# thowell/IterativeLQR.jl

Hardware: AMD Instinct MI355X
Metric: trajectories/sec (whole node), acrobot T=101 batch=1024/GPU (higher is better)
Workload: dtype f64

## Files before the change

iterativelqr.jl_amd/csrc/ilqr_device.hpp:

```cpp
#pragma once

#include <hip/hip_runtime.h>

#include "../../include/ilqr_hip.h"
#include "ilqr_layout.hpp"
#include "ilqr_math.hpp"
#include "ilqr_launch_plan.hpp"
#include "ilqr_ric_schedule.hpp"

namespace ilqr {

struct KArgs {
    double* ws;
    Layout L;
    int B;
    int constrained;
    int stage;
    ilqr_options opt;
    const double* x1;
    const double* u_in;
    double* trace;
    int trace_cap;
    double* qv;
    QLayout QL;
// ... 125 lines not shown
    double *lds;
    double *trace;
    int trace_cap, trace_len;
    double *Q;
    QLayout QL;
    double delta;
    double delta_next;
    int delta_next_ok;
    const double* gzero;
    int T, N, C, lane, wave;
    double objective, max_violation, step_size, gradient_norm;
    int status, iterations, outer_iterations, potrf_info, rollouts, states_eq_nominal;
    int cost_par;
#ifdef ILQR_PROFILE
    double prof[PROF_N];
#endif
};

template <class M> __device__ void gradients_large(Inst<M>& I, bool constrained);
template <class M> __device__ void cost_pass_large(Inst<M>& I, bool at_states, bool upd_J, bool upd_viol, bool constrained, double& J_out, double& viol_out);
template <class M> __device__ void reset_model_objective_large(Inst<M>& I, bool literal);
template <class M, bool STORE_VALUE> __device__ void backward_pass_large(Inst<M>& I);
template <class M> __device__ void rollout_large(Inst<M>& I, double alpha, bool want_delta, double& delta_out);

template <class M, bool STAGE, int NC>
__device__ __forceinline__ double objective_term(double l, const double (&cv)[NC], const double* lam, const double* rho, double* act, bool with_al) {
#pragma clang fp contract(off)
    if (!with_al) return l;
    double dot = 0.0, pen = 0.0;
#pragma unroll
    for (int i = 0; i < NC; ++i) {
        const double lm = lam[i];
        const bool ineq = STAGE ? IneqMask<M>::s(i) : IneqMask<M>::t(i);
        const bool inactive = ineq && cv[i] < 0.0 && lm == 0.0;
        act[i] = inactive ? 0.0 : 1.0;
        dot = __builtin_fma(lm, cv[i], dot);
        const double c2 = cv[i] * cv[i], hr = 0.5 * rho[i];
        if (!inactive) pen = __builtin_fma(hr, c2, pen);
    }
    return (l + dot) + pen;
}
__device__ __forceinline__ void al_multipliers(double rho, double act, double lam, double c, double& ir, double& ct) {
#pragma clang fp contract(off)
    ir = rho * act;
    ct = __builtin_fma(ir, c, lam);
}
struct ObjAcc {
    double a0 = 0.0, a1 = 0.0, a2 = 0.0, a3 = 0.0;
    __device__ __forceinline__ void add(int t, double v) {
        const int q = (t >> 4) & 3;
        a0 += q == 0 ? v : 0.0; a1 += q == 1 ? v : 0.0; a2 += q == 2 ? v : 0.0; a3 += q == 3 ? v : 0.0;
    }
    __device__ __forceinline__ double S() const { return (a0 + a2) + (a1 + a3); }
};

template <class M>
__device__ void cost_pass(Inst<M>& I, const double* X, const double* U, bool upd_J, bool upd_viol,
                          bool constrained, double& J_out, double& viol_out) {
    constexpr int n = M::NX, m = M::NU, ncs = M::NCS, nct = M::NCT;
    ILQR_PROF_BEGIN();
    double Jp = 0.0, vp = 0.0;
    constexpr bool PARK = waves_of<M>::value == 2;
    const int t_first = (PARK && I.wave != 0) ? I.T : I.lane;
    for (int t = t_first; t < I.T; t += 64) {
        double w[cdim<M::NW>::v];
        load_w<M::NW>(I.w, t, w);
        double xt[n];
#pragma unroll
        for (int i = 0; i < n; ++i) xt[i] = X[t * n + i];
        if (t < I.N) {
            double ut[m];
#pragma unroll
            for (int i = 0; i < m; ++i) ut[i] = U[t * m + i];
            double l_ = 0.0;
            if (upd_J) { l_ = M::cost_s(xt, ut, w); ILQR_OPAQUE(l_); }
            if constexpr (ncs == 0) { if (upd_J) Jp += l_; }
            if constexpr (ncs > 0) {
                if (!constrained) { if (upd_J) Jp += l_; }
                if (constrained) {
                    double cv[ncs];
                    M::con_s(xt, ut, w, cv);
                    const int off = t * ncs;
                    if (upd_J) { double v_ = objective_term<M, true, ncs>(l_, cv, I.lam + off, I.rho + off, I.act + off, true); ILQR_OPAQUE(v_); Jp += v_; }
                    if (upd_viol) {
#pragma unroll
                        for (int i = 0; i < ncs; ++i) {
                            I.c[off + i] = cv[i];
                            const bool ineq = IneqMask<M>::s(i);
                            vp = nanmax(vp, ineq ? nanmax(0.0, cv[i]) : fabs(cv[i]));
                        }
                    }
                }
            }
        } else {
            double l_ = 0.0;
            if (upd_J) { l_ = M::cost_t(xt, w); ILQR_OPAQUE(l_); }
            if constexpr (nct == 0) { if (upd_J) Jp += l_; }
            if constexpr (nct > 0) {
                if (!constrained) { if (upd_J) Jp += l_; }
                if (constrained) {
                    double cv[nct];
                    M::con_t(xt, w, cv);
                    const int off = I.N * ncs;
                    if (upd_J) { double v_ = objective_term<M, false, nct>(l_, cv, I.lam + off, I.rho + off, I.act + off, true); ILQR_OPAQUE(v_); Jp += v_; }
                    if (upd_viol) {
#pragma unroll
                        for (int i = 0; i < nct; ++i) {
                            I.c[off + i] = cv[i];
                            const bool ineq = IneqMask<M>::t(i);
                            vp = nanmax(vp, ineq ? nanmax(0.0, cv[i]) : fabs(cv[i]));
                        }
                    }
                }
            }
        }
    }
    if constexpr (PARK) {
        double* hand = I.zs + 8 + 2 * I.cost_par;
        I.cost_par ^= 1;
        if (I.wave == 0) {
            J_out = wave_sum(Jp);
            viol_out = wave_max(vp);
            if (I.lane == 0) { hand[0] = J_out; hand[1] = viol_out; }
        }
        __syncthreads();
        if (I.wave != 0) { J_out = hand[0]; viol_out = hand[1]; }
    } else {
        J_out = wave_sum(Jp);
        viol_out = wave_max(vp);
        __syncthreads();
    }
#ifndef ILQR_PROFILE_BAR
    ILQR_PROF_END(I, PROF_COST);
#endif
}

template <class M>
__device__ void cost_bang(Inst<M>& I, bool mode_current, bool constrained) {
    const bool one_pass = mode_current || I.states_eq_nominal || !constrained;
    const int npass = one_pass ? 1 : 2;
    for (int pass = 0; pass < npass; ++pass) {
        const bool at_states = mode_current || pass == 1;
        const bool upd_J = pass == 0;
        const bool upd_viol = one_pass || pass == 1;
        double J, v;
        if constexpr (is_large<M>::value) cost_pass_large<M>(I, at_states, upd_J, upd_viol, constrained, J, v);
        else cost_pass<M>(I, at_states ? I.x : I.xb, at_states ? I.u : I.ub, upd_J, upd_viol, constrained, J, v);
        if (upd_J) I.objective = J;
        if (upd_viol && constrained) I.max_violation = v;
    }
}

template <class M>
__device__ void gradients_small(Inst<M>& I, bool constrained) {
    constexpr int n = M::NX, m = M::NU, ncs = M::NCS, nct = M::NCT, W = waves_of<M>::value;
    ILQR_PROF_BEGIN();
    for (int t = I.lane + 64 * I.wave; t < I.T; t += 64 * W) {
        double w[cdim<M::NW>::v];
        load_w<M::NW>(I.w, t, w);
        double xt[n];
#pragma unroll
        for (int i = 0; i < n; ++i) xt[i] = I.xb[t * n + i];
        if (t < I.N) {
            double ut[m];
#pragma unroll
            for (int i = 0; i < m; ++i) ut[i] = I.ub[t * m + i];
            {
                double fx[n * n], fu[n * m];
                M::dyn_jac(xt, ut, w, fx, fu);
#pragma unroll
                for (int i = 0; i < n * n; ++i) I.fx[t * n * n + i] = fx[i];
#pragma unroll
                for (int i = 0; i < n * m; ++i) I.fu[t * n * m + i] = fu[i];
            }
            double gx[n], gu[m];
            M::cost_s_grad(xt, ut, w, gx, gu);
            if constexpr (ncs == 0) {
                M::cost_s_hess_acc(xt, ut, w, I.gxx + t * n * n, I.guu + t * m * m, I.gux + t * m * n);
#pragma unroll
                for (int i = 0; i < n; ++i) I.gx[t * n + i] = gx[i];
#pragma unroll
                for (int i = 0; i < m; ++i) I.gu[t * m + i] = gu[i];
                continue;
            }
            M::cost_s_hess_acc(xt, ut, w, I.gxx + t * n * n, I.guu + t * m * m, I.gux + t * m * n);
            if constexpr (ncs > 0) {
                if (constrained) {
                    double ct[ncs], ir[ncs];
                    const int off = t * ncs;
#pragma unroll
                    for (int i = 0; i < ncs; ++i) al_multipliers(I.rho[off + i], I.act[off + i], I.lam[off + i], I.c[off + i], ir[i], ct[i]);
                    M::al_s(xt, ut, w, ct, ir, gx, gu, I.gxx + t * n * n, I.guu + t * m * m, I.gux + t * m * n);
                }
            }
#pragma unroll
            for (int i = 0; i < n; ++i) I.gx[t * n + i] = gx[i];
#pragma unroll
            for (int i = 0; i < m; ++i) I.gu[t * m + i] = gu[i];
        } else {
            double gx[n];
            M::cost_t_grad(xt, w, gx);
            M::cost_t_hess_acc(xt, w, I.gxx + t * n * n);
            if constexpr (nct > 0) {
                if (constrained) {
                    double ct[nct], ir[nct];
                    const int off = I.N * ncs;
#pragma unroll
                    for (int i = 0; i < nct; ++i) al_multipliers(I.rho[off + i], I.act[off + i], I.lam[off + i], I.c[off + i], ir[i], ct[i]);
                    M::al_t(xt, w, ct, ir, gx, I.gxx + t * n * n);
                }
            }
#pragma unroll
            for (int i = 0; i < n; ++i) I.gx[t * n + i] = gx[i];
        }
    }
    __syncthreads();
    ILQR_PROF_END(I, PROF_GRAD);
}

template <int m>
__device__ __forceinline__ int potrf_U(double (&A)[m * m], double (&R)[m]) {
    int info = 0;
#pragma unroll
    for (int j = 0; j < m; ++j) {
        double ajj = A[j * m + j];
#pragma unroll
        for (int l = 0; l < j; ++l) ajj -= A[j * m + l] * A[j * m + l];
        const bool ok = (info == 0) && (ajj > 0.0);
        const bool fail_now = (info == 0) && !(ajj > 0.0);
        info = fail_now ? j + 1 : info;
        double dq, rq;
        sqrt_rsqrt_fast(ok ? ajj : 1.0, dq, rq);
        const double dbad = fail_now ? ajj : A[j * m + j];
        const double d = ok ? dq : dbad;
        A[j * m + j] = d;
        double r = rq;
        if (__builtin_expect(!ok, 0)) r = 1.0 / dbad;
        R[j] = r;
#pragma unroll
        for (int c = j + 1; c < m; ++c) {
            double v = A[c * m + j];
#pragma unroll
            for (int l = 0; l < j; ++l) v -= A[j * m + l] * A[c * m + l];
            A[c * m + j] = ok ? v * r : A[c * m + j];
        }
    }
    return info;
}
template <int m>
__device__ __forceinline__ int potrf_U(double (&A)[m * m]) {
    double R[m];
    return potrf_U<m>(A, R);
}
template <int m>
__device__ __forceinline__ bool potrf_U_nofail(double (&A)[m * m], double (&R)[m]) {
    bool bad = false;
#pragma unroll
    for (int j = 0; j < m; ++j) {
        double ajj = A[j * m + j];
#pragma unroll
        for (int l = 0; l < j; ++l) ajj -= A[j * m + l] * A[j * m + l];
        bad |= !(ajj > 0.0);
        double dq, rq;
        sqrt_rsqrt_fast(ajj, dq, rq);
        A[j * m + j] = dq;
        R[j] = rq;
#pragma unroll
        for (int c = j + 1; c < m; ++c) {
            double v = A[c * m + j];
#pragma unroll
            for (int l = 0; l < j; ++l) v -= A[j * m + l] * A[c * m + l];
            A[c * m + j] = v * rq;
        }
    }
    return bad;
}
template <int m, int nrhs>
__device__ __forceinline__ void potrs_U_rdiag(const double (&U)[m * m], const double (&R)[m], double (&B)[m * nrhs]) {
#pragma unroll
    for (int c = 0; c < nrhs; ++c) {
#pragma unroll
        for (int i = 0; i < m; ++i) {
            double v = B[c * m + i];
#pragma unroll
            for (int l = 0; l < i; ++l) v -= U[i * m + l] * B[c * m + l];
            B[c * m + i] = v * R[i];
        }
#pragma unroll
        for (int i = m - 1; i >= 0; --i) {
            double v = B[c * m + i];
#pragma unroll
            for (int l = i + 1; l < m; ++l) v -= U[l * m + i] * B[c * m + l];
            B[c * m + i] = v * R[i];
        }
    }
}
template <int m, int nrhs>
__device__ __forceinline__ void potrs_U(const double (&U)[m * m], double (&B)[m * nrhs]) {
#pragma unroll
    for (int c = 0; c < nrhs; ++c) {
#pragma unroll
        for (int i = 0; i < m; ++i) {
            double v = B[c * m + i];
#pragma unroll
            for (int l = 0; l < i; ++l) v -= U[i * m + l] * B[c * m + l];
            B[c * m + i] = v / U[i * m + i];
        }
#pragma unroll
        for (int i = m - 1; i >= 0; --i) {
            double v = B[c * m + i];
#pragma unroll
            for (int l = i + 1; l < m; ++l) v -= U[l * m + i] * B[c * m + l];
            B[c * m + i] = v / U[i * m + i];
        }
    }
}

__device__ __forceinline__ double lane_bcast(double v, int src_lane) {
    int lo = __double2loint(v), hi = __double2hiint(v);
    lo = __builtin_amdgcn_readlane(lo, src_lane);
    hi = __builtin_amdgcn_readlane(hi, src_lane);
    return __hiloint2double(hi, lo);
}
__device__ __forceinline__ double row_from_next_quad(double v) {
    int lo = __double2loint(v), hi = __double2hiint(v), olo, ohi;
    asm volatile("s_nop 7\n\ts_nop 7\n\tv_mov_b32_dpp %0, %2 row_shl:4 row_mask:0xf bank_mask:0xf bound_ctrl:1\n\t"
                 "v_mov_b32_dpp %1, %3 row_shl:4 row_mask:0xf bank_mask:0xf bound_ctrl:1\n\ts_nop 1"
// ... 570 lines not shown
        }
        return __builtin_amdgcn_ballot_w64(!(qmin > 0.0) || P != P) != 0;
    } else {
        unsigned agx = vr ? lds(I.gx + tl * n + r) : zero;             const unsigned dgx = vr ? 32u * n : 0u;
        unsigned agu = lds(I.gu + tl);
        unsigned aK = vr ? lds(I.K + tl * n + r) : zero;
        unsigned arq = vr ? lds(I.ring + M1_RQ + r) : zero;            const unsigned dq = vr ? 32u * n : 0u;
        unsigned asa = lds(I.ring + M1_RS);
        unsigned ak = lds(I.k + tl);
        asm volatile("" : "+v"(agu), "+v"(asa), "+v"(ak));
        unsigned oLu = goff(I.gbase + I.hLu + tl);
        unsigned oLx = vr ? goff(I.gbase + I.hLx + tl * n + r) : goff(I.gzero + 2 + GZERO_REGION);   const unsigned dLx = vr ? 32u * n : 0u;
        auto GS = [&](unsigned o, int off, double v) { *(double*)(const_cast<char*>(gb) + (size_t)o + (ptrdiff_t)(8 * off)) = v; };
        double p = vr ? I.gx[N * n + r] : 0.0;
        if (STORE_VALUE && b0 && vr && c == 0) I.p[N * n + r] = p;
        double gmax = 0.0, nu = 0.0, dacc = 0.0;
        unsigned long long nanmask = 0;
        auto fetch = [&](Opnd& o, int i) {
            o.fx = LD(afx, i * n * n); o.fu = LD(afu, i * n);
            o.c0 = LD(agx, i * n); o.c1 = LD(agu, i);
        };
        auto step = [&](const Opnd& o, int i) {
            ILQR_ISA_MARK("riccati_step", ROLE);
            const double Qx = mfma444(o.fx, p, o.c0);
            const double Qu = mfma444(o.fu, p, o.c1);
            const double sa = LD(asa, i * n);
            const double Kc = LD(aK, i * n), Quxc = LD(arq, i * n), uxtc = LD(arq, M1_RU - M1_RQ + i * n);
            const double k = (Qu * sa) * -1.0;
            const double pn = fma(uxtc, k, fma(Quxc, k, fma(Kc, Qu, Qx)));
            const double Lx = Qx - pn;
            asm("v_max_f64 %0, %1, |%2|" : "=v"(gmax) : "v"(gmax), "v"(Lx));
            asm("v_max_f64 %0, %1, |%2| ; %3" : "=v"(gmax) : "v"(gmax), "v"(Qu), "v"(Lx));
            nanmask |= __builtin_amdgcn_ballot_w64(__builtin_isunordered(Lx, Qu));
            ST(ak, i, k); GS(oLu, i, Qu); GS(oLx, i * n, Lx);
            const double wv = mfma444(o.fu, nu, Qu);
            dacc = fma(wv, k, dacc);
            const double nun = mfma444(o.fx, nu, Lx);
            nu = fma(Kc, wv, nun);
            if constexpr (STORE_VALUE) {
                if (b0 && c == 0) {
                    if (vr) I.p[t * n + r] = pn;
                    if (I.Q != nullptr) {
                        if (vr) I.Q[I.QL.Qx + t * n + r] = Qx;
                        if (r == 0) I.Q[I.QL.Qu + t] = Qu;
                    }
                }
            }
            p = pn;
            --t;
        };
        if (t0 & 1) fetch(A, t0 & 3); else fetch(B, t0 & 3);
        for (int e = t0 & 3;; e = 3) {
            ILQR_BAR_BEGIN();
            __syncthreads();
            ILQR_BAR_END(I, PROF_COST);
            switch (e) {
                case 3: fetch(B, 2); step(A, 3); [[fallthrough]];
                case 2: fetch(A, 1); step(B, 2); [[fallthrough]];
                case 1: fetch(B, 0); step(A, 1); [[fallthrough]];
                default:
                    afx -= dfx; afu -= dfu; agx -= dgx; agu -= 32u;
                    fetch(A, 3); step(B, 0);
            }
            aK -= dq; ak -= 32u; oLu -= 32u; oLx -= dLx;
            arq += par ? (0u - dq) : dq;
            asa += par ? (unsigned)(-32 * n) : 32u * n;
            par ^= 1;
            asm volatile("" : "+v"(afx), "+v"(afu), "+v"(agx), "+v"(agu), "+v"(aK), "+v"(ak), "+v"(arq), "+v"(asa));
            if (t < 0) break;
        }
        I.gradient_norm = wave_max(nanmask != 0 ? __builtin_nan("") : gmax);
        I.delta_next = lane_bcast(dacc, 0);
#ifdef ILQR_PROFILE_BAR
        if (lane == 0) I.zs[7] += I.prof[PROF_COST];
        I.prof[PROF_COST] = 0.0;
#endif
        return false;
    }
}

template <class M, bool STORE_VALUE>
__device__ __forceinline__ void backward_pass(Inst<M>& I) {
    ILQR_PROF_BEGIN();
    if constexpr (is_large<M>::value) backward_pass_large<M, STORE_VALUE>(I);
    else {
        if constexpr (waves_of<M>::value == 1) {
            backward_pass_mfma<M, STORE_VALUE, 0>(I);
            __syncthreads();
        } else {
            bool literal = true;
            if constexpr (M::NU == 1) {
                if (I.wave == 0) {
                    const bool bad = backward_pass_m1<M, STORE_VALUE, 1>(I);
                    if (I.lane == 0) { I.zs[6] = bad ? 1.0 : 0.0; I.zs[3] = (double)I.potrf_info; }
                } else {
                    backward_pass_m1<M, STORE_VALUE, 2>(I);
                    if (I.lane == 0) { I.zs[2] = I.gradient_norm; I.zs[5] = I.delta_next; }
                }
                __syncthreads();
                literal = I.zs[6] != 0.0;
#ifdef ILQR_PROFILE
                if (literal) I.prof[PROF_DELTA] += 1.0;
#endif
                if (literal) {
                    if (I.wave == 0 && I.lane == 0) I.scal[S_LITERAL_PASSES] += 1.0;
                    __syncthreads();
                }
            }
            if (literal) {
                if (I.wave == 0) {
                    backward_pass_split<M, STORE_VALUE, 1>(I);
                    if (I.lane == 0) I.zs[3] = (double)I.potrf_info;
                } else {
                    backward_pass_split<M, STORE_VALUE, 2>(I);
                    if (I.lane == 0) { I.zs[2] = I.gradient_norm; I.zs[5] = I.delta_next; }
                }
                __syncthreads();
                if constexpr (lagrangian_home_is_hbm<M>::value) {
                    for (int i = threadIdx.x; i < I.N * M::NX; i += 128) I.gbase[I.hLx + i] = I.Lx[i];
                    for (int i = threadIdx.x; i < I.N * M::NU; i += 128) I.gbase[I.hLu + i] = I.Lu[i];
                }
            }
            I.gradient_norm = I.zs[2]; I.potrf_info = (int)I.zs[3];
            I.delta_next = I.zs[5]; I.delta_next_ok = 1;
        }
    }
    ILQR_PROF_END(I, PROF_BACKWARD);
}

template <class M, bool MULTI = false>
__device__ void rollout_small(Inst<M>& I, double alpha, bool with_delta, double& delta_out, int nt = 1, double* buf1 = nullptr,
                              int xs = 0, int bsz = 0) {
    constexpr int n = M::NX, m = M::NU;
    constexpr bool MF = (n <= 4 && m <= 4) && waves_of<M>::value == 1;
    constexpr bool PRE = (m <= n);
    typedef __attribute__((address_space(3))) double ldsd;
    const int lane = I.lane;
    double* xr = I.x; double* ur = I.u;
    const double alpha0 = alpha;
    (void)alpha0;
    if constexpr (MULTI) {
        const int jr = (lane >> 4) < nt - 1 ? (lane >> 4) : nt - 1;
        if (jr > 0) { xr = buf1 + (jr - 1) * bsz; ur = xr + xs; }
        for (int j = 0; j < jr; ++j) alpha *= 0.5;
    }
    if constexpr (PRE) {
        for (int t = lane; t < I.N; t += 64) {
#pragma unroll
            for (int i = 0; i < m; ++i) {
                double b = 0.0;
#pragma unroll
                for (int j = 0; j < n; ++j) b = fma(I.K[t * m * n + j * m + i], I.xb[t * n + j], b);
                if constexpr (MULTI) {
                    double al = alpha0;
                    for (int j = 0; j < nt; ++j) {
                        double* xj = j == 0 ? I.x : buf1 + (j - 1) * bsz;
                        double* uj = j == 0 ? I.u : xj + xs;
                        uj[t * m + i] = fma(I.k[t * m + i], al, I.ub[t * m + i]);
                        xj[(t + 1) * n + i] = b;
                        al *= 0.5;
                    }
                } else {
                    const double a = fma(I.k[t * m + i], alpha, I.ub[t * m + i]);
                    I.u[t * m + i] = a;
                    I.x[(t + 1) * n + i] = b;
                }
            }
        }
        __builtin_amdgcn_fence(__ATOMIC_RELEASE, "wavefront");
        __builtin_amdgcn_wave_barrier();
    }
    double xt[n];
#pragma unroll
    for (int i = 0; i < n; ++i) xt[i] = I.xb[i];
#pragma unroll
    for (int i = 0; i < n; ++i) xr[i] = xt[i];
    const int r = lane >> 4, c = lane & 3, blk = (lane >> 2) & 3;
    const bool vnn = r < n && c < n, vnm = r < n && c < m, vmn = r < m && c < n;
    const bool vn1 = c == 0 && r < n, vm1 = c == 0 && r < m;
    double zx = 0.0, dacc = 0.0;
    (void)blk;
    const typename M::WaveCtx wcx = M::template wave_ctx<ILQR_PIN_ROLLOUT_CONSTANTS>(lane);
    unsigned aK = (unsigned)(size_t)(ldsd*)I.K, aU = (unsigned)(size_t)(ldsd*)ur, aX = (unsigned)(size_t)(ldsd*)xr;
    unsigned aKb = (unsigned)(size_t)(ldsd*)I.k, aUb = (unsigned)(size_t)(ldsd*)I.ub, aXb = (unsigned)(size_t)(ldsd*)I.xb;
    asm volatile("" : "+v"(aK), "+v"(aU), "+v"(aX));
    if constexpr (!PRE) asm volatile("" : "+v"(aKb), "+v"(aUb), "+v"(aXb));
    auto L = [](unsigned a, int off) -> double { return *(const ldsd*)(size_t)(a + 8u * off); };
    auto S = [](unsigned a, int off, double v) { *(ldsd*)(size_t)(a + 8u * off) = v; };
    struct Ops { double K[m * n], a[m], b[m], xb[PRE ? 1 : n]; };
    auto fetch = [&](Ops& o, int d) {
#pragma unroll
        for (int i = 0; i < m * n; ++i) o.K[i] = L(aK, d * m * n + i);
        if constexpr (PRE) {
#pragma unroll
            for (int i = 0; i < m; ++i) { o.a[i] = L(aU, d * m + i); o.b[i] = L(aX, (d + 1) * n + i); }
        } else {
#pragma unroll
            for (int i = 0; i < m; ++i) { o.a[i] = L(aKb, d * m + i); o.b[i] = L(aUb, d * m + i); }
#pragma unroll
            for (int i = 0; i < n; ++i) o.xb[i] = L(aXb, d * n + i);
        }
    };
    const double* pKT = (MF && vnm) ? I.K + r * m + c : I.zs;     const int sKT = (MF && vnm) ? m * n : 0;
    const double* zsrc = slim_of<M>::value ? I.gzero : I.zs;
    const double* pfxT = (MF && vnn) ? I.fx + r * n + c : zsrc;   const int sfxT = (MF && vnn) ? n * n : 0;
    const double* pfuT = (MF && vmn) ? I.fu + r * n + c : zsrc;   const int sfuT = (MF && vmn) ? n * m : 0;
    const double* pkc = (MF && vm1) ? I.k + r : I.zs;             const int skc = (MF && vm1) ? m : 0;
    const double* pLx = (MF && vn1) ? I.Lx + r : I.zs;            const int sLx = (MF && vn1) ? n : 0;
    const double* pLu = (MF && vm1) ? I.Lu + r : I.zs;
    auto step = [&](const Ops& o, int t, int d, const double (&xin)[n], double (&xout)[n]) {
        ILQR_ISA_MARK("rollout_step", MF ? 1 : 0);
        double KT = 0.0, fxT = 0.0, fuT = 0.0, kc = 0.0, Lxc = 0.0, Luc = 0.0;
        if constexpr (MF) {
            if (with_delta) {
                KT = *pKT; fxT = *pfxT; fuT = *pfuT; kc = *pkc; Lxc = *pLx; Luc = *pLu;
                pKT += sKT; pfxT += sfxT; pfuT += sfuT; pkc += skc; pLx += sLx; pLu += skc;
            }
        }
        double ut[m];
#pragma unroll
        for (int i = 0; i < m; ++i) {
            double a1 = 0.0;
#pragma unroll
            for (int j = 0; j < n; ++j) a1 = fma(o.K[j * m + i], xin[j], a1);
            if constexpr (PRE) {
                ut[i] = (o.a[i] + a1) - o.b[i];
            } else {
                double a2 = 0.0;
#pragma unroll
                for (int j = 0; j < n; ++j) a2 = fma(o.K[j * m + i], o.xb[j], a2);
                ut[i] = (fma(o.a[i], alpha, o.b[i]) + a1) - a2;
            }
        }
        double zu = 0.0, fz = 0.0;
        if constexpr (MF) {
            if (with_delta) {
                zu = mfma444(KT, zx, kc);
                fz = mfma444(fxT, zx, 0.0);
                dacc = mfma444(Lxc, zx, dacc);
            }
        }
        double w[cdim<M::NW>::v];
        load_w<M::NW>(I.w, t, w);
        M::dyn_wave(wcx, lane, xin, ut, w, xout);
#pragma unroll
        for (int i = 0; i < m; ++i) S(aU, d * m + i, ut[i]);
#pragma unroll
        for (int i = 0; i < n; ++i) S(aX, (d + 1) * n + i, xout[i]);
        if constexpr (MF) {
            if (with_delta) {
                dacc = mfma444(Luc, zu, dacc);
                zx = mfma444(fuT, zu, fz);
            }
        }
    };
    auto advance2 = [&]() {
        aK += 16u * m * n; aU += 16u * m; aX += 16u * n;
        if constexpr (!PRE) { aKb += 16u * m; aUb += 16u * m; aXb += 16u * n; }
    };
    Ops A, B;
    double xo[n];
    if (I.N > 0) fetch(A, 0);
    int t = 0;
    for (int pairs = I.N >> 1; pairs > 0; --pairs, t += 2) {
        fetch(B, 1);
        step(A, t, 0, xt, xo);
        fetch(A, 2);
        step(B, t + 1, 1, xo, xt);
        advance2();
    }
    if (t < I.N) {
        step(A, t, 0, xt, xo);
#pragma unroll
        for (int i = 0; i < n; ++i) xt[i] = xo[i];
    }
    if constexpr (MF) {
        if (with_delta) delta_out = lane_bcast(dacc, 0);
    }
}

template <class M>
__device__ double delta_small(Inst<M>& I) {
    constexpr int n = M::NX, m = M::NU;
    double zx[n], d = 0.0;
#pragma unroll
    for (int i = 0; i < n; ++i) zx[i] = 0.0;
    for (int t = 0; t < I.N; ++t) {
        ILQR_ISA_MARK("delta_step", 0);
        double du[m];
#pragma unroll
        for (int i = 0; i < m; ++i) {
            double acc = 0.0;
#pragma unroll
            for (int j = 0; j < n; ++j) acc += I.K[t * m * n + j * m + i] * zx[j];
            du[i] = I.k[t * m + i] + acc;
        }
#pragma unroll
        for (int j = 0; j < n; ++j) d += I.Lx[t * n + j] * zx[j];
#pragma unroll
        for (int i = 0; i < m; ++i) d += I.Lu[t * m + i] * du[i];
        double zn[n];
#pragma unroll
        for (int i = 0; i < n; ++i) {
            double a1 = 0.0, a2 = 0.0;
#pragma unroll
            for (int j = 0; j < m; ++j) a1 += I.fu[t * n * m + j * n + i] * du[j];
#pragma unroll
            for (int j = 0; j < n; ++j) a2 += I.fx[t * n * n + j * n + i] * zx[j];
            zn[i] = a1 + a2;
        }
#pragma unroll
        for (int i = 0; i < n; ++i) zx[i] = zn[i];
    }
    return d;
}

}
#include "ilqr_device_large.hpp"
namespace ilqr {

template <class M>
__device__ __forceinline__ void gradients(Inst<M>& I, bool constrained) {
    if constexpr (is_large<M>::value) gradients_large<M>(I, constrained);
    else gradients_small<M>(I, constrained);
}
template <class M, bool MULTI = false>
__device__ __forceinline__ void rollout_bang(Inst<M>& I, double alpha, bool with_delta, double& delta_out, int nt = 1,
                                             double* buf1 = nullptr, int xs = 0, int bsz = 0) {
    if constexpr (is_large<M>::value) rollout_large<M>(I, alpha, with_delta, delta_out);
    else {
        ILQR_PROF_BEGIN();
        if constexpr (waves_of<M>::value == 1) {
            rollout_small<M>(I, alpha, with_delta, delta_out);
            __syncthreads();
        } else {
            if (I.wave == 0) {
                double unused = 0.0;
                if constexpr (MULTI) rollout_small<M, true>(I, alpha, false, unused, nt, buf1, xs, bsz);
                else rollout_small<M>(I, alpha, false, unused);
            } else if (with_delta && !I.delta_next_ok) {
                const double d = delta_small<M>(I);
                if (I.lane == 0) I.zs[4] = d;
            }
            __syncthreads();
            if (with_delta) delta_out = I.delta_next_ok ? I.delta_next : I.zs[4];
        }
        I.rollouts += 1;
        I.states_eq_nominal = 0;
        ILQR_PROF_END(I, PROF_ROLLOUT);
    }
}

template <class M, int SPEC = 0>
__device__ void forward_pass(Inst<M>& I, const ilqr_options& opt, bool constrained) {
    constexpr int n = M::NX, m = M::NU;
    constexpr bool MF = true;
    constexpr bool SP = SPEC != 0 && !is_large<M>::value && waves_of<M>::value == 2;
    const double c1 = 1.0e-4;
    const int max_iterations = 25;
    I.status = 0;
    const double J_prev = I.objective;
    double delta = 0.0;
    I.delta = 0.0;
    I.step_size = 1.0;
    int iteration = 1;
    const int xs = (I.T * n + 1) & ~1, bsz = xs + ((I.N * m + 1) & ~1);
    const int region = ((I.N * n * n + 1) & ~1) + ((I.N * n * m + 1) & ~1);
    const int nb = SP ? (region / bsz < 3 ? region / bsz : 3) : 0;
    double* const buf1 = I.fx;
    double* const home = I.gbase + (I.fx - I.lds);
    bool saved = false;
    int last = 0;
    auto accept = [&](const double* X, const double* U) {
        constexpr int CS = 64 * waves_of<M>::value;
        const int c0 = is_large<M>::value ? (int)threadIdx.x : I.lane + 64 * I.wave;
        for (int i = c0; i < I.T * n; i += CS) I.xb[i] = X[i];
        for (int i = c0; i < I.N * m; i += CS) I.ub[i] = U[i];
        I.states_eq_nominal = 1;
        I.status = 1;
    };
    while (I.step_size >= opt.min_step_size) {
        if (iteration > max_iterations) break;
        const bool want_delta = MF && iteration == 1 && opt.line_search == 1;
        int nt = 1;
        if constexpr (SP) {
            if (iteration >= (SPEC == 2 ? 1 : 2) && (!want_delta || I.delta_next_ok)) {
                double s = 0.5 * I.step_size;
                while (nt < 1 + nb && s >= opt.min_step_size && iteration + nt <= max_iterations) { nt += 1; s *= 0.5; }
            }
            if (nt > 1 && !saved) {
                for (int i = (int)threadIdx.x; i < nb * bsz; i += 128) home[i] = buf1[i];
                saved = true;
                __syncthreads();
            }
        }
        double d = 0.0;
        rollout_bang<M, SP>(I, I.step_size, want_delta, d, nt, buf1, xs, bsz);
        if (want_delta) { delta = d; I.delta = d; }
        bool done = false;
        for (int j = 0; j < nt; ++j) {
            double* const xs0 = I.x; double* const us0 = I.u;
            if (j > 0) { I.rollouts += 1; I.x = buf1 + (j - 1) * bsz; I.u = I.x + xs; }
            cost_bang<M>(I, true, constrained);
            const double* X = I.x; const double* U = I.u;
            I.x = xs0; I.u = us0;
            last = j;
            if (I.objective <= J_prev + c1 * I.step_size * delta) {
                accept(X, U);
                done = true;
                break;
            }
            I.step_size *= 0.5;
            iteration += 1;
        }
        if (done) break;
    }
    if (I.status || last > 0) __syncthreads();
    if constexpr (SP) {
        if (last > 0) {
            const double* X = buf1 + (last - 1) * bsz;
            for (int i = (int)threadIdx.x; i < I.T * n; i += 128) I.x[i] = X[i];
            for (int i = (int)threadIdx.x; i < I.N * m; i += 128) I.u[i] = X[xs + i];
            __syncthreads();
        }
        if (saved && (!I.status || opt.line_search == 0)) {
            for (int i = (int)threadIdx.x; i < nb * bsz; i += 128) buf1[i] = home[i];
            __syncthreads();
        }
    }
}

template <class M>
__device__ __forceinline__ void zero_lagrangian_gradient(Inst<M>& I) {
    for (int i = I.lane; i < I.N * M::NX; i += 64) I.Lx[i] = 0.0;
    for (int i = I.lane; i < I.N * M::NU; i += 64) I.Lu[i] = 0.0;
    if constexpr (lagrangian_home_is_hbm<M>::value) {
        for (int i = I.lane; i < I.N * M::NX; i += 64) I.gbase[I.hLx + i] = 0.0;
        for (int i = I.lane; i < I.N * M::NU; i += 64) I.gbase[I.hLu + i] = 0.0;
    }
}

template <class M>
__device__ void reset_model_objective(Inst<M>& I, bool literal = true) {
    constexpr int n = M::NX, m = M::NU;
    if constexpr (is_large<M>::value) {
        reset_model_objective_large<M>(I, literal);
        return;
    }
    for (int i = I.lane; i < I.N * n * n; i += 64) I.fx[i] = 0.0;
    for (int i = I.lane; i < I.N * n * m; i += 64) I.fu[i] = 0.0;
    for (int i = I.lane; i < I.T * n; i += 64) I.gx[i] = 0.0;
    for (int i = I.lane; i < I.N * m; i += 64) I.gu[i] = 0.0;
    for (int i = I.lane; i < I.T * n * n; i += 64) I.gxx[i] = 0.0;
    for (int i = I.lane; i < I.N * m * m; i += 64) I.guu[i] = 0.0;
    for (int i = I.lane; i < I.N * m * n; i += 64) I.gux[i] = 0.0;
    __syncthreads();
}

__device__ __forceinline__ void dual_update_row(double& lam, double& rho, double c, bool ineq, const ilqr_options& opt) {
#pragma clang fp contract(off)
    double l = __builtin_fma(rho, c, lam);
    if (ineq) l = nanmax(0.0, l);
    lam = l;
    const double r = opt.scaling_penalty * rho;
    rho = (r < opt.max_penalty || r != r) ? r : opt.max_penalty;
}
template <class M>
__device__ void al_update(Inst<M>& I, const ilqr_options& opt) {
    constexpr int ncs = M::NCS, W = waves_of<M>::value;
    for (int i = I.lane + 64 * I.wave; i < I.C; i += 64 * W) {
        const int ns = I.N * ncs;
        bool ineq;
        if (i < ns) ineq = ncs > 0 ? IneqMask<M>::s(i % (ncs > 0 ? ncs : 1)) : false;
        else ineq = IneqMask<M>::t(i - ns);
        double lam = I.lam[i], rho = I.rho[i];
        dual_update_row(lam, rho, I.c[i], ineq, opt);
        I.lam[i] = lam; I.rho[i] = rho;
    }
    __syncthreads();
}

template <class M, bool STORE_VALUE, int SPEC = 0>
__device__ void solve_loops(Inst<M>& I, const ilqr_options& opt, bool constrained, bool al_outer, int o_start = 1, int it_start = 0,
                            double obj_prev0 = 0.0, bool warm_duals = false) {
    if (al_outer && o_start == 1 && it_start == 0) {
        I.objective = 0.0; I.max_violation = 0.0; I.status = 0; I.iterations = 0; I.gradient_norm = 0.0;
        zero_lagrangian_gradient<M>(I);
        if (!warm_duals) for (int i = I.lane; i < I.C; i += 64) {
            I.lam[i] = 0.0;
            I.rho[i] = opt.initial_constraint_penalty;
        }
        __syncthreads();
        I.outer_iterations = 0;
    }
    const int outer_max = al_outer ? opt.max_dual_updates : 1;
    for (int o = o_start; o <= outer_max; ++o) {
        if (al_outer) I.outer_iterations = o;
        const bool mid = it_start > 0 && o == o_start;
        if (!mid) {
            reset_model_objective<M>(I, false);
            if (opt.reset_cache) {
                I.objective = 0.0; I.max_violation = 0.0; I.status = 0; I.iterations = 0;
            }
        }
        double obj_prev = mid ? obj_prev0 : 0.0;
        for (int it = mid ? it_start : 0; it <= opt.max_iterations; ++it) {
            if (it == 0) cost_bang<M>(I, false, constrained);
            else forward_pass<M, SPEC>(I, opt, constrained);
            if (it == 0 || opt.line_search != 0) {
                gradients<M>(I, constrained);
                backward_pass<M, STORE_VALUE>(I);
            }
            if (it == 0) { obj_prev = I.objective; continue; }
            I.iterations += 1;
            if (I.trace != nullptr && I.trace_len < I.trace_cap && I.lane == 0) {
                double* r = I.trace + (size_t)I.trace_len * TRACE_W;
                r[0] = (double)(al_outer ? o : I.outer_iterations); r[1] = (double)it; r[2] = I.objective; r[3] = I.gradient_norm;
                r[4] = I.max_violation; r[5] = I.step_size; r[6] = (double)I.status; r[7] = (double)I.rollouts;
            }
            I.trace_len += 1;
            if (I.gradient_norm < opt.lagrangian_gradient_tolerance) break;
            if (fabs(I.objective - obj_prev) < opt.objective_tolerance) break;
            obj_prev = I.objective;
            if (!I.status) break;
        }
        if (!al_outer) break;
        cost_bang<M>(I, false, true);
        if (I.max_violation <= opt.constraint_tolerance) break;
        al_update<M>(I, opt);
    }
}

template <class M>
__device__ __forceinline__ void inst_setup(Inst<M>& I, const KArgs& a, double* smem, int b, int swap_roles = 0) {
    const Layout& L = a.L;
    double* g = a.ws + (size_t)b * (size_t)L.stride;
    I.xb = smem + L.xb; I.ub = smem + L.ub; I.x = smem + L.x; I.u = smem + L.u;
    I.fx = smem + L.fx; I.fu = smem + L.fu; I.gx = smem + L.gx; I.gu = smem + L.gu;
    I.K = smem + L.K; I.k = smem + L.k; I.Lx = smem + L.Lx; I.Lu = smem + L.Lu;
    I.c = smem + L.c; I.lam = smem + L.lam; I.rho = smem + L.rho; I.act = smem + L.act;
    I.zs = smem + L.zslot; I.gzero = g + L.gzero; I.w = smem + L.w; I.ring = smem + L.ring;
    I.gxx = g + L.gxx; I.guu = g + L.guu; I.gux = g + L.gux; I.P = g + L.P; I.p = g + L.p; I.scal = g + L.scal;
    I.T = L.T; I.N = L.T - 1; I.C = L.C; I.lane = threadIdx.x & 63; I.wave = (int)(threadIdx.x >> 6) ^ swap_roles;
    I.cost_par = 0;
    I.lds = smem; I.gbase = g; I.fv_off = 0; I.hc_off = 0; I.hLx = L.Lx; I.hLu = L.Lu;
    I.trace = a.trace ? a.trace + (size_t)b * (size_t)a.trace_cap * TRACE_W : nullptr;
    I.trace_cap = a.trace_cap; I.trace_len = 0;
    I.Q = a.qv ? a.qv + (size_t)b * (size_t)a.QL.stride : nullptr; I.QL = a.QL;
    I.delta = I.scal[S_DELTA]; I.delta_next = 0.0; I.delta_next_ok = 0;
    if constexpr (is_large<M>::value) {
        I.xb = g + L.xb; I.ub = g + L.ub; I.x = g + L.x; I.u = g + L.u;
        I.fx = g + L.fx; I.fu = g + L.fu; I.gx = g + L.gx; I.gu = g + L.gu;
        I.K = g + L.K; I.k = g + L.k; I.Lx = g + L.Lx; I.Lu = g + L.Lu;
        I.c = g + L.c; I.lam = g + L.lam; I.rho = g + L.rho; I.act = g + L.act;
        I.zs = g + L.zslot; I.w = g + L.w;
        I.fv_off = L.fv; I.hc_off = L.hc;
        if (threadIdx.x == 0) store_layout_lds<M>(L);
    } else {
        const double2* src = reinterpret_cast<const double2*>(g);
        double2* dst = reinterpret_cast<double2*>(smem);
        const int nd = slim_of<M>::value ? L.lds_doubles_slim : L.lds_doubles;
        for (int i = I.lane + 64 * I.wave; i < nd / 2; i += 64 * waves_of<M>::value) dst[i] = src[i];
        __syncthreads();
        if (I.lane == 0 && I.wave == 0) { I.zs[0] = 0.0; I.zs[1] = 0.0; }
#ifdef ILQR_PROFILE_BAR
        if (I.lane == 0 && I.wave == 0) I.zs[7] = 0.0;
#endif
        if constexpr (slim_of<M>::value) { I.fx = g + L.fx; I.fu = g + L.fu; }
    }
    I.objective = I.scal[S_OBJECTIVE]; I.max_violation = I.scal[S_MAX_VIOLATION];
    I.step_size = I.scal[S_STEP_SIZE]; I.gradient_norm = I.scal[S_GRADIENT_NORM];
    I.status = (int)I.scal[S_STATUS]; I.iterations = (int)I.scal[S_ITERATIONS];
    I.outer_iterations = (int)I.scal[S_OUTER_ITERATIONS]; I.potrf_info = (int)I.scal[S_POTRF_INFO];
    I.rollouts = (int)I.scal[S_ROLLOUTS]; I.states_eq_nominal = (int)I.scal[S_STATES_EQ_NOMINAL];
#ifdef ILQR_PROFILE
    for (int i = 0; i < PROF_N; ++i) I.prof[i] = 0.0;
#endif
    __syncthreads();
}

template <class M>
// ... 430 lines not shown
```

Baseline: 44150.

## Recompute dynamics Jacobians instead of saving/restoring speculative line-search buffers

The speculative multi-step line search reuses the fx/fu Jacobian region in LDS as scratch for extra rollouts. Before, that region was copied out to global memory and copied back when the line search failed. Now the copies are dropped, and on failure the Jacobians are recomputed from the nominal trajectory. Speculation is also turned off when line_search is 0, and the pre-rollout pointer arithmetic is simplified by hoisting the k/ub loads. This trades a global-memory round trip on every speculative iteration for a recompute that only happens on line-search failure.

```diff
diff --git a/iterativelqr.jl_amd/csrc/ilqr_device.hpp b/iterativelqr.jl_amd/csrc/ilqr_device.hpp
--- a/iterativelqr.jl_amd/csrc/ilqr_device.hpp
+++ b/iterativelqr.jl_amd/csrc/ilqr_device.hpp
@@ -301,6 +301,32 @@
 }
 
 template <class M>
+__device__ __forceinline__ void dynamics_jacobian_step(Inst<M>& I, int t, const double (&xt)[M::NX], const double (&ut)[M::NU],
+                                                       const double (&w)[cdim<M::NW>::v]) {
+    constexpr int n = M::NX, m = M::NU;
+    double fx[n * n], fu[n * m];
+    M::dyn_jac(xt, ut, w, fx, fu);
+#pragma unroll
+    for (int i = 0; i < n * n; ++i) I.fx[t * n * n + i] = fx[i];
+#pragma unroll
+    for (int i = 0; i < n * m; ++i) I.fu[t * n * m + i] = fu[i];
+}
+template <class M>
+__device__ void dynamics_jacobians_small(Inst<M>& I) {
+    constexpr int n = M::NX, m = M::NU, W = waves_of<M>::value;
+    for (int t = I.lane + 64 * I.wave; t < I.N; t += 64 * W) {
+        double w[cdim<M::NW>::v];
+        load_w<M::NW>(I.w, t, w);
+        double xt[n], ut[m];
+#pragma unroll
+        for (int i = 0; i < n; ++i) xt[i] = I.xb[t * n + i];
+#pragma unroll
+        for (int i = 0; i < m; ++i) ut[i] = I.ub[t * m + i];
+        dynamics_jacobian_step<M>(I, t, xt, ut, w);
+    }
+    __syncthreads();
+}
+template <class M>
 __device__ void gradients_small(Inst<M>& I, bool constrained) {
     constexpr int n = M::NX, m = M::NU, ncs = M::NCS, nct = M::NCT, W = waves_of<M>::value;
     ILQR_PROF_BEGIN();
@@ -314,14 +340,7 @@
             double ut[m];
 #pragma unroll
             for (int i = 0; i < m; ++i) ut[i] = I.ub[t * m + i];
-            {
-                double fx[n * n], fu[n * m];
-                M::dyn_jac(xt, ut, w, fx, fu);
-#pragma unroll
-                for (int i = 0; i < n * n; ++i) I.fx[t * n * n + i] = fx[i];
-#pragma unroll
-                for (int i = 0; i < n * m; ++i) I.fu[t * n * m + i] = fu[i];
-            }
+            dynamics_jacobian_step<M>(I, t, xt, ut, w);
             double gx[n], gu[m];
             M::cost_s_grad(xt, ut, w, gx, gu);
             if constexpr (ncs == 0) {
@@ -1198,13 +1217,16 @@
 #pragma unroll
                 for (int j = 0; j < n; ++j) b = fma(I.K[t * m * n + j * m + i], I.xb[t * n + j], b);
                 if constexpr (MULTI) {
+                    const double kt = I.k[t * m + i], ubt = I.ub[t * m + i];
                     double al = alpha0;
+                    double* xj = I.x + (t + 1) * n + i;
+                    double* uj = I.u + t * m + i;
                     for (int j = 0; j < nt; ++j) {
-                        double* xj = j == 0 ? I.x : buf1 + (j - 1) * bsz;
-                        double* uj = j == 0 ? I.u : xj + xs;
-                        uj[t * m + i] = fma(I.k[t * m + i], al, I.ub[t * m + i]);
-                        xj[(t + 1) * n + i] = b;
+                        *uj = fma(kt, al, ubt);
+                        *xj = b;
                         al *= 0.5;
+                        xj = buf1 + j * bsz + (t + 1) * n + i;
+                        uj = buf1 + j * bsz + xs + t * m + i;
                     }
                 } else {
                     const double a = fma(I.k[t * m + i], alpha, I.ub[t * m + i]);
@@ -1414,8 +1436,7 @@
     const int region = ((I.N * n * n + 1) & ~1) + ((I.N * n * m + 1) & ~1);
     const int nb = SP ? (region / bsz < 3 ? region / bsz : 3) : 0;
     double* const buf1 = I.fx;
-    double* const home = I.gbase + (I.fx - I.lds);
-    bool saved = false;
+    bool used = false;
     int last = 0;
     auto accept = [&](const double* X, const double* U) {
         constexpr int CS = 64 * waves_of<M>::value;
@@ -1430,15 +1451,11 @@
         const bool want_delta = MF && iteration == 1 && opt.line_search == 1;
         int nt = 1;
         if constexpr (SP) {
-            if (iteration >= (SPEC == 2 ? 1 : 2) && (!want_delta || I.delta_next_ok)) {
+            if (iteration >= (SPEC == 2 ? 1 : 2) && opt.line_search != 0 && (!want_delta || I.delta_next_ok)) {
                 double s = 0.5 * I.step_size;
                 while (nt < 1 + nb && s >= opt.min_step_size && iteration + nt <= max_iterations) { nt += 1; s *= 0.5; }
             }
-            if (nt > 1 && !saved) {
-                for (int i = (int)threadIdx.x; i < nb * bsz; i += 128) home[i] = buf1[i];
-                saved = true;
-                __syncthreads();
-            }
+            used = used || nt > 1;
         }
         double d = 0.0;
         rollout_bang<M, SP>(I, I.step_size, want_delta, d, nt, buf1, xs, bsz);
@@ -1469,10 +1486,7 @@
             for (int i = (int)threadIdx.x; i < I.N * m; i += 128) I.u[i] = X[xs + i];
             __syncthreads();
         }
-        if (saved && (!I.status || opt.line_search == 0)) {
-            for (int i = (int)threadIdx.x; i < nb * bsz; i += 128) buf1[i] = home[i];
-            __syncthreads();
-        }
+        if (used && !I.status) dynamics_jacobians_small<M>(I);
     }
 }
 
```

Result: no change. 44140 (-0.0%).
